# ayotoasset/AdditiveCausalExpansion

Measured on NVIDIA B200. Metric: nadam_iters_per_sec, higher is better.
Workload: dtype f64

## Files before the change

additivecausalexpansion_b200/csrc/uut_i8.cuh:

```cuda
#pragma once
#include "common.cuh"

namespace ace {

namespace oz {
constexpr int NMOD = 16;
constexpr int MOD[NMOD] = {256, 255, 253, 251, 247, 241, 239, 233, 229, 227, 223, 217, 211, 199, 197, 193};
constexpr int BM = 128, BN = 256, BK = 32;
constexpr int CPB = TB / BK;
constexpr int STAGES = 8;
constexpr int A_BYTES = BM * BK, B_BYTES = BN * BK;
constexpr int STAGE_BYTES = A_BYTES + B_BYTES;
constexpr size_t SMEM_BYTES = 1024 + (size_t)STAGES * STAGE_BYTES + 128;
static_assert(2 * SMEM_BYTES <= 227 * 1024 && 3 * SMEM_BYTES > 228 * 1024, "exactly two CTAs per SM");
constexpr int TMEM_COLS = BN;
constexpr int THREADS = 192;
constexpr int MAX_N = 65408;
static_assert((long)128 * 128 * MAX_N <= 2147483647L, "INT32 accumulators may overflow");
constexpr uint32_t IDESC = (2u << 4) | (1u << 7) | (1u << 10) | ((uint32_t)(BN >> 3) << 17) | ((uint32_t)(BM >> 4) << 24);

constexpr int crt_bits(int n_pad) { return n_pad <= 16384 ? 55 : 54; }
constexpr unsigned __int128 crt_half_range() {
  unsigned __int128 p = 1;
  for (int t = 0; t < NMOD; ++t) p *= (unsigned)MOD[t];
  return p / 2;
}
static_assert(((unsigned __int128)16384 << (2 * 55)) < crt_half_range(), "CRT range at b = 55");
static_assert(((unsigned __int128)MAX_N << (2 * 54)) < crt_half_range(), "CRT range at b = 54");

__host__ __device__ inline size_t block_off(int nb, int t, int rb, int c) {
  const long nc = (long)nb * CPB;
  const long per_plane = (long)nb * nc - (long)CPB * nb * (nb - 1) / 2;
  const long off = (long)rb * nc - (long)CPB * rb * (rb - 1) / 2 + (c - (long)CPB * rb);
  return ((size_t)t * per_plane + off) * (size_t)(BM * BK);
}
__host__ __device__ inline size_t slot_bytes(int nb) { return block_off(nb, 1, 0, 0); }
inline size_t plane_bytes(int nb) { return block_off(nb, NMOD + 1, 0, 0); }
__host__ __device__ inline size_t res_off(int ti, int tj) { return ((size_t)ti * (ti + 1) / 2 + tj) * (size_t)(TB * TB); }
inline long product_tiles(int nb) { return (long)(nb / 2) * (nb / 2 + 1) + (nb & 1) * (nb / 2 + 1); }

struct Tables {
  int m[NMOD];
  unsigned magic[NMOD];
  int c14[NMOD], c28[NMOD], c42[NMOD];
  float mf[NMOD], rcp[NMOD];
  float inv[NMOD];
  float w[NMOD][NMOD];
  unsigned long long p8;
};

inline Tables make_tables() {
  Tables T{};
  for (int k = 0; k < NMOD; ++k) {
    const long m = MOD[k];
    T.m[k] = (int)m;
    T.magic[k] = (unsigned)(((1ull << 32) + (unsigned long long)m - 1) / (unsigned long long)m);
    T.c14[k] = (int)((1L << 14) % m);
    T.c28[k] = (int)((1L << 28) % m);
    T.c42[k] = (int)((1L << 42) % m);
    T.mf[k] = (float)m;
    T.rcp[k] = 1.0f / (float)m;
    long pk = 1;
    for (int j = 0; j < k; ++j) pk = pk * MOD[j] % m;
    long inv = 1;
    while (k > 0 && pk * inv % m != 1) ++inv;
    T.inv[k] = (float)inv;
    long pj = 1;
    for (int j = 0; j < k; ++j) {
      T.w[k][j] = (float)(pj * inv % m);
      pj = pj * MOD[j] % m;
    }
  }
  T.p8 = 1;
  for (int j = 0; j < 8; ++j) T.p8 *= (unsigned long long)MOD[j];
  return T;
}
}

__device__ __forceinline__ int oz_smod(unsigned x, const oz::Tables& T, int t) {
  const int r = (int)(x - (unsigned)T.m[t] * __umulhi(x, T.magic[t]));
  return r > (T.m[t] >> 1) ? r - T.m[t] : r;
}

__device__ __forceinline__ uint64_t oz_smem_desc(uint32_t saddr) {
  return (uint64_t)((saddr >> 4) & 0x3FFF) | ((uint64_t)(128 >> 4) << 16) | ((uint64_t)(256 >> 4) << 32) |
         (1ull << 46);
}

__device__ __forceinline__ void tc_fence_before() { asm volatile("tcgen05.fence::before_thread_sync;" ::: "memory"); }
__device__ __forceinline__ void tc_fence_after() { asm volatile("tcgen05.fence::after_thread_sync;" ::: "memory"); }

__device__ __forceinline__ void tc_mma_i8(uint32_t d_tmem, uint64_t adesc, uint64_t bdesc, uint32_t accumulate) {
  asm volatile(
      "{\n.reg .pred p;\nsetp.ne.b32 p, %4, 0;\n"
      "tcgen05.mma.cta_group::1.kind::i8 [%0], %1, %2, %3, p;\n}\n" ::"r"(d_tmem),
      "l"(adesc), "l"(bdesc), "r"(oz::IDESC), "r"(accumulate)
      : "memory");
}

__device__ __forceinline__ void tc_commit(uint64_t* bar) {
  asm volatile("tcgen05.commit.cta_group::1.mbarrier::arrive::one.shared::cluster.b64 [%0];" ::"r"(smem_u32(bar))
               : "memory");
}

__device__ __forceinline__ void tc_ld16(uint32_t taddr, uint32_t (&v)[16]) {
  asm volatile(
      "tcgen05.ld.sync.aligned.32x32b.x16.b32 {%0,%1,%2,%3,%4,%5,%6,%7,%8,%9,%10,%11,%12,%13,%14,%15}, [%16];"
      : "=r"(v[0]), "=r"(v[1]), "=r"(v[2]), "=r"(v[3]), "=r"(v[4]), "=r"(v[5]), "=r"(v[6]), "=r"(v[7]), "=r"(v[8]),
        "=r"(v[9]), "=r"(v[10]), "=r"(v[11]), "=r"(v[12]), "=r"(v[13]), "=r"(v[14]), "=r"(v[15])
      : "r"(taddr)
      : "memory");
}

__device__ __forceinline__ double oz_u(const double* A, long ld, const double* DU, int rb, int cb, int r, int kk) {
  return (cb == rb) ? DU[(size_t)rb * TB * TB + r + (size_t)kk * TB] : A[(size_t)rb * TB + r + (size_t)(cb * TB + kk) * ld];
}

__global__ void __launch_bounds__(128) oz_rowmax_kernel(const double* __restrict__ A, long ld,
                                                        const double* __restrict__ DU,
                                                        unsigned long long* __restrict__ rowmax) {
  const int cb = blockIdx.x, rb = blockIdx.y, r = threadIdx.x;
  if (cb < rb) return;
  double m = 0.0;
#pragma unroll 8
  for (int kk = 0; kk < TB; ++kk) m = fmax(m, fabs(oz_u(A, ld, DU, rb, cb, r, kk)));
  atomicMax(rowmax + rb * TB + r, (unsigned long long)__double_as_longlong(m));
}

__global__ void __launch_bounds__(128) oz_split_kernel(const double* __restrict__ A, long ld,
                                                       const double* __restrict__ DU,
                                                       const unsigned long long* __restrict__ rowmax, int nb, int b,
                                                       const __grid_constant__ oz::Tables T,
                                                       int8_t* __restrict__ planes, int* __restrict__ ex) {
  using namespace oz;
  const int cb = blockIdx.x, rb = blockIdx.y, r = threadIdx.x;
  if (cb < rb) return;
  const double m = __longlong_as_double((long long)rowmax[rb * TB + r]);
  int e = 0;
  if (m > 0.0) frexp(m, &e);
  if (cb == rb) ex[rb * TB + r] = e;
  const double scale = ldexp(1.0, b - e);
#pragma unroll 1
  for (int q = 0; q < TB / 16; ++q) {
    uint32_t w[NMOD][4];
#pragma unroll
    for (int t = 0; t < NMOD; ++t) w[t][0] = w[t][1] = w[t][2] = w[t][3] = 0u;
#pragma unroll
    for (int x16 = 0; x16 < 16; ++x16) {
      const long long a = __double2ll_rn(rint(oz_u(A, ld, DU, rb, cb, r, q * 16 + x16) * scale));
      const unsigned long long ua = (unsigned long long)(a < 0 ? -a : a);
      const unsigned q0 = (unsigned)ua & 0x3FFFu, q1 = (unsigned)(ua >> 14) & 0x3FFFu,
                     q2 = (unsigned)(ua >> 28) & 0x3FFFu, q3 = (unsigned)(ua >> 42);
      const int sh = 8 * (x16 & 3);
      w[0][x16 >> 2] |= ((uint32_t)a & 0xffu) << sh;
#pragma unroll
      for (int t = 1; t < NMOD; ++t) {
        const int s = oz_smod(q0 + q1 * (unsigned)T.c14[t] + q2 * (unsigned)T.c28[t] + q3 * (unsigned)T.c42[t], T, t);
        w[t][x16 >> 2] |= ((uint32_t)(a < 0 ? -s : s) & 0xffu) << sh;
      }
    }
    const int c = cb * CPB + q / 2;
    const size_t in_blk = (size_t)(r >> 3) * 256 + (q & 1) * 128 + (r & 7) * 16;
#pragma unroll
    for (int t = 0; t < NMOD; ++t)
      *reinterpret_cast<uint4*>(planes + block_off(nb, t + 1, rb, c) + in_blk) =
          make_uint4(w[t][0], w[t][1], w[t][2], w[t][3]);
  }
}

__global__ void __launch_bounds__(oz::THREADS, 2) uut_i8_mod_kernel(int8_t* __restrict__ planes, int nb, int slot,
                                                                    int m, double inv_m) {
  using namespace oz;
  extern __shared__ unsigned char smem_raw[];
  unsigned char* sm = reinterpret_cast<unsigned char*>((reinterpret_cast<uintptr_t>(smem_raw) + 1023) & ~uintptr_t(1023));
  uint64_t* full = reinterpret_cast<uint64_t*>(sm + (size_t)STAGES * STAGE_BYTES);
  uint64_t* empty = full + STAGES;
  uint64_t* done = empty + STAGES;
  uint32_t* tmem_slot = reinterpret_cast<uint32_t*>(done + 1);
  const int warp = threadIdx.x >> 5, lane = threadIdx.x & 31;

  int ti, tj2;
  {
    const long L = blockIdx.x;
    long q = (long)((sqrt(4.0 * (double)L + 1.0) - 1.0) * 0.5);
    while (q * (q + 1) > L) --q;
    while ((q + 1) * (q + 2) <= L) ++q;
    const long rem = L - q * (q + 1);
    ti = (int)(2 * q + rem / (q + 1));
    tj2 = (int)(rem % (q + 1));
  }
  const int jb0 = 2 * tj2;
  const bool has1 = jb0 + 1 <= ti;
  const int jb1 = has1 ? jb0 + 1 : jb0;
  const int c_begin = ti * CPB, nchunks = nb * CPB - c_begin;
  const int8_t* src = planes;

  if (threadIdx.x == 0) {
    for (int s = 0; s < STAGES; ++s) {
      mbar_init(&full[s], 1);
      mbar_init(&empty[s], 1);
    }
    mbar_init(done, 1);
    fence_mbar_init();
  }
  if (warp == 1) {
    asm volatile("tcgen05.alloc.cta_group::1.sync.aligned.shared::cta.b32 [%0], %1;" ::"r"(smem_u32(tmem_slot)),
                 "r"(TMEM_COLS)
                 : "memory");
    asm volatile("tcgen05.relinquish_alloc_permit.cta_group::1.sync.aligned;" ::: "memory");
  }
  tc_fence_before();
  __syncthreads();
  tc_fence_after();
  const uint32_t tmem = *tmem_slot;

  if (warp == 0) {
    if (lane == 0) {
      for (int it = 0; it < nchunks; ++it) {
        const int s = it % STAGES;
        mbar_wait(&empty[s], ((it / STAGES) & 1) ^ 1);
        mbar_arrive_expect_tx(&full[s], STAGE_BYTES);
        unsigned char* st = sm + (size_t)s * STAGE_BYTES;
        const int c = c_begin + it;
        tma_bulk_g2s(st, src + block_off(nb, slot + 1, ti, c), A_BYTES, &full[s]);
        tma_bulk_g2s(st + A_BYTES, src + block_off(nb, slot + 1, jb0, c), A_BYTES, &full[s]);
        tma_bulk_g2s(st + 2 * A_BYTES, src + block_off(nb, slot + 1, jb1, c), A_BYTES, &full[s]);
      }
    }
    __syncwarp();
  } else if (warp == 1) {
    if (lane == 0) {
      for (int it = 0; it < nchunks; ++it) {
        const int s = it % STAGES;
        mbar_wait(&full[s], (it / STAGES) & 1);
        tc_fence_after();
        const uint32_t a0 = smem_u32(sm + (size_t)s * STAGE_BYTES);
        tc_mma_i8(tmem, oz_smem_desc(a0), oz_smem_desc(a0 + A_BYTES), it > 0 ? 1u : 0u);
        tc_commit(&empty[s]);
      }
      tc_commit(done);
    }
    __syncwarp();
  } else {
    mbar_wait(done, 0);
    tc_fence_after();
    const int q = warp & 3;
    const int r = q * 32 + lane;
    const uint32_t trow = tmem + ((uint32_t)(q * 32) << 16);
    int8_t* dst = planes + block_off(nb, slot, 0, 0) + (size_t)r * TB;
#pragma unroll 1
    for (int jc = 0; jc < (has1 ? BN : TB) / 32; ++jc) {
      uint32_t v[2][16];
      tc_ld16(trow + (uint32_t)(jc * 32), v[0]);
      tc_ld16(trow + (uint32_t)(jc * 32 + 16), v[1]);
      asm volatile("tcgen05.wait::ld.sync.aligned;" ::: "memory");
      uint32_t pk[8];
#pragma unroll
      for (int j = 0; j < 32; ++j) {
        const int x = (int)v[j >> 4][j & 15];
        int res;
        if (m == 256) {
          res = x;
        } else {
          res = x - m * (int)rint((double)x * inv_m);
        }
        if ((j & 3) == 0) pk[j >> 2] = 0u;
        pk[j >> 2] |= ((uint32_t)res & 0xffu) << (8 * (j & 3));
      }
      uint4* o = reinterpret_cast<uint4*>(dst + res_off(ti, jb0 + (jc >> 2)) + (jc & 3) * 32);
      o[0] = make_uint4(pk[0], pk[1], pk[2], pk[3]);
      o[1] = make_uint4(pk[4], pk[5], pk[6], pk[7]);
    }
  }
  tc_fence_before();
  __syncthreads();
  if (warp == 1) {
    tc_fence_after();
    asm volatile("tcgen05.dealloc.cta_group::1.sync.aligned.b32 %0, %1;" ::"r"(tmem), "r"(TMEM_COLS) : "memory");
  }
}

__device__ __forceinline__ float oz_i2f(int x) { return __int_as_float(0x4B400000 + x) - 0x1.8p23f; }
__device__ __forceinline__ int oz_f2i(float x) { return __float_as_int(x + 0x1.8p23f) - 0x4B400000; }

__device__ __forceinline__ double oz_crt(const int (&res)[oz::NMOD], const oz::Tables& T, int scale_exp) {
  using namespace oz;
  float v[NMOD];
  v[0] = oz_i2f(res[0]);
#pragma unroll
  for (int k = 1; k < NMOD; ++k) {
    float s = oz_i2f(res[k]) * T.inv[k];
#pragma unroll
    for (int j = 0; j < k; ++j) s = fmaf(-v[j], T.w[k][j], s);
    float r = fmaf(-T.mf[k], rintf(s * T.rcp[k]), s);
    const float h = 0.5f * T.mf[k];
    r = r > h ? r - T.mf[k] : r;
    r = r < -h ? r + T.mf[k] : r;
    v[k] = r;
  }
  unsigned long long ulo = (unsigned long long)(long long)oz_f2i(v[7]);
  unsigned long long uhi = (unsigned long long)(long long)oz_f2i(v[NMOD - 1]);
#pragma unroll
  for (int k = 6; k >= 0; --k) ulo = ulo * (unsigned)T.m[k] + (unsigned long long)(long long)oz_f2i(v[k]);
#pragma unroll
  for (int k = NMOD - 2; k >= 8; --k) uhi = uhi * (unsigned)T.m[k] + (unsigned long long)(long long)oz_f2i(v[k]);
  const __int128 x = (__int128)(long long)uhi * (__int128)T.p8 + (__int128)(long long)ulo;
  const bool neg = x < 0;
  const unsigned __int128 u = neg ? (unsigned __int128)(-x) : (unsigned __int128)x;
  const unsigned long long hi = (unsigned long long)(u >> 64), lo = (unsigned long long)u;
  double d;
  if (hi == 0) {
    d = ldexp(__ull2double_rn(lo), scale_exp);
  } else {
    const int z = __clzll((long long)hi);
    const unsigned long long top = z ? (hi << z) | (lo >> (64 - z)) : hi;
    const unsigned long long rest = lo << z;
    d = ldexp(__ull2double_rn(top | (rest != 0 ? 1ull : 0ull)), scale_exp + 64 - z);
  }
  return neg ? -d : d;
}

__global__ void __launch_bounds__(256) oz_crt_kernel(const int8_t* __restrict__ planes, const int* __restrict__ ex,
                                                     int nb, int b, const __grid_constant__ oz::Tables T,
                                                     double* __restrict__ C, long ldc) {
  using namespace oz;
  __shared__ double tile[32][TB + 1];
  int ti, tj;
  {
    const long L = blockIdx.x;
    long t = (long)((sqrt(8.0 * (double)L + 1.0) - 1.0) * 0.5);
    while (t * (t + 1) / 2 > L) --t;
    while ((t + 1) * (t + 2) / 2 <= L) ++t;
    ti = (int)t;
    tj = (int)(L - t * (t + 1) / 2);
  }
  const size_t sb = slot_bytes(nb);
  const int8_t* blk = planes + res_off(ti, tj);
  const int tid = threadIdx.x, rr = tid >> 3, c0 = (tid & 7) * 16;
  const int i0 = ti * TB, j0 = tj * TB;
#pragma unroll 1
  for (int r0 = 0; r0 < TB; r0 += 32) {
    const int r = r0 + rr;
    uint4 rv[NMOD];
#pragma unroll
    for (int t = 0; t < NMOD; ++t) rv[t] = *reinterpret_cast<const uint4*>(blk + t * sb + (size_t)r * TB + c0);
    const int ei = ex[i0 + r];
#pragma unroll 1
    for (int j = 0; j < 16; ++j) {
      int res[NMOD];
#pragma unroll
      for (int t = 0; t < NMOD; ++t) {
        const uint32_t wv = j < 4 ? rv[t].x : j < 8 ? rv[t].y : j < 12 ? rv[t].z : rv[t].w;
        res[t] = (int)(int8_t)(wv >> (8 * (j & 3)));
      }
      tile[rr][c0 + j] = oz_crt(res, T, ei + ex[j0 + c0 + j] - 2 * b);
    }
    __syncthreads();
#pragma unroll 4
    for (int k = tid; k < 32 * TB; k += 256) {
      const int a = k >> 7, c = k & (TB - 1);
      C[(size_t)(i0 + r0 + a) * ldc + j0 + c] = tile[a][c];
    }
    if (ti != tj) {
#pragma unroll 4
      for (int k = tid; k < 32 * TB; k += 256) {
        const int c = k >> 5, a = k & 31;
        C[(size_t)(j0 + c) * ldc + i0 + r0 + a] = tile[a][c];
      }
    }
    __syncthreads();
  }
}

struct OzWork {
  int8_t* planes = nullptr;
  unsigned long long* rowmax = nullptr;
  int* ex = nullptr;
};

inline int configure_uut_i8_kernel() {
  ACE_CUDA(cudaFuncSetAttribute(uut_i8_mod_kernel, cudaFuncAttributeMaxDynamicSharedMemorySize, (int)oz::SMEM_BYTES));
  return 0;
}

inline int launch_uut_i8(const OzWork& o, const double* A, const double* DU, int nb, double* C, cudaStream_t st) {
  using namespace oz;
  if ((long)nb * TB > MAX_N) {
    set_error("uut_i8: n_pad beyond the CRT range bound");
    return -2;
  }
  if (!o.planes || !o.rowmax || !o.ex) {
    set_error("uut_i8: residue-plane workspace not allocated");
    return -2;
  }
  static const Tables T = make_tables();
  const long ld = (long)nb * TB;
  const int b = crt_bits((int)ld);
  ACE_CUDA(cudaMemsetAsync(o.rowmax, 0, sizeof(unsigned long long) * (size_t)ld, st));
  const dim3 g2(nb, nb);
  oz_rowmax_kernel<<<g2, TB, 0, st>>>(A, ld, DU, o.rowmax);
  ACE_CUDA(cudaGetLastError());
  oz_split_kernel<<<g2, TB, 0, st>>>(A, ld, DU, o.rowmax, nb, b, T, o.planes, o.ex);
  ACE_CUDA(cudaGetLastError());
  const long tiles = product_tiles(nb);
  for (int t = 0; t < NMOD; ++t) {
    uut_i8_mod_kernel<<<(unsigned)tiles, THREADS, SMEM_BYTES, st>>>(o.planes, nb, t, MOD[t], 1.0 / MOD[t]);
    ACE_CUDA(cudaGetLastError());
  }
  oz_crt_kernel<<<(unsigned)((long)nb * (nb + 1) / 2), 256, 0, st>>>(o.planes, o.ex, nb, b, T, C, ld);
  ACE_CUDA(cudaGetLastError());
  return 0;
}

}
```

Baseline: 8.075.

## Compute residues with paired fp32 FMA magic-number rounding in split and mod kernels

Replaces the integer magic-division modular reductions in the residue split kernel and the fp64 rint-based reduction in the TMEM epilogue with packed float2 FMA arithmetic. Values are decomposed into 14-bit pieces via fp64 magic-constant tricks, combined with signed residue constants and reduced using a biased round-to-nearest, so the low byte of the float bits is the residue. Bytes are packed with byte_perm instead of shift/or loops. This is meant to cut integer-multiply and fp64 cost in these phases, at the risk of subtle exactness errors if fp32 intermediate ranges are exceeded.

```diff
diff --git a/additivecausalexpansion_b200/csrc/uut_i8.cuh b/additivecausalexpansion_b200/csrc/uut_i8.cuh
--- a/additivecausalexpansion_b200/csrc/uut_i8.cuh
+++ b/additivecausalexpansion_b200/csrc/uut_i8.cuh
@@ -41,8 +41,8 @@
 
 struct Tables {
   int m[NMOD];
-  unsigned magic[NMOD];
-  int c14[NMOD], c28[NMOD], c42[NMOD];
+  float2 s_c14[NMOD], s_c28[NMOD], s_c42[NMOD];
+  float2 s_rcp[NMOD], s_nm[NMOD];
   float mf[NMOD], rcp[NMOD];
   float inv[NMOD];
   float w[NMOD][NMOD];
@@ -54,10 +54,12 @@
   for (int k = 0; k < NMOD; ++k) {
     const long m = MOD[k];
     T.m[k] = (int)m;
-    T.magic[k] = (unsigned)(((1ull << 32) + (unsigned long long)m - 1) / (unsigned long long)m);
-    T.c14[k] = (int)((1L << 14) % m);
-    T.c28[k] = (int)((1L << 28) % m);
-    T.c42[k] = (int)((1L << 42) % m);
+    auto smod = [m](long x) { x %= m; return (float)(x > m / 2 ? x - m : x); };
+    T.s_c14[k] = make_float2(smod(1L << 14), smod(1L << 14));
+    T.s_c28[k] = make_float2(smod(1L << 28), smod(1L << 28));
+    T.s_c42[k] = make_float2(smod(1L << 42), smod(1L << 42));
+    T.s_rcp[k] = make_float2(1.0f / (float)m, 1.0f / (float)m);
+    T.s_nm[k] = make_float2(-(float)m, -(float)m);
     T.mf[k] = (float)m;
     T.rcp[k] = 1.0f / (float)m;
     long pk = 1;
@@ -77,9 +79,14 @@
 }
 }
 
-__device__ __forceinline__ int oz_smod(unsigned x, const oz::Tables& T, int t) {
-  const int r = (int)(x - (unsigned)T.m[t] * __umulhi(x, T.magic[t]));
-  return r > (T.m[t] >> 1) ? r - T.m[t] : r;
+constexpr float OZ_MAGIC = 0x1.8p23f;
+__device__ __forceinline__ float oz_i2f(int x) { return __int_as_float(0x4B400000 + x) - OZ_MAGIC; }
+__device__ __forceinline__ int oz_f2i(float x) { return __float_as_int(x + OZ_MAGIC) - 0x4B400000; }
+__device__ __forceinline__ float2 oz_f2(float x) { return make_float2(x, x); }
+
+__device__ __forceinline__ float2 oz_smod2_biased(float2 s, float2 rcp, float2 nm) {
+  const float2 q = __fadd2_rn(__ffma2_rn(s, rcp, oz_f2(OZ_MAGIC)), oz_f2(-OZ_MAGIC));
+  return __fadd2_rn(__ffma2_rn(q, nm, s), oz_f2(OZ_MAGIC));
 }
 
 __device__ __forceinline__ uint64_t oz_smem_desc(uint32_t saddr) {
@@ -127,6 +134,17 @@
   atomicMax(rowmax + rb * TB + r, (unsigned long long)__double_as_longlong(m));
 }
 
+__device__ __forceinline__ void oz_pieces(double v, float (&p)[4], uint32_t& low) {
+  const double th = fma(v, 0x1p-28, 0x1.8p52);
+  const int hi = __double2loint(th);
+  const int lo = __double2loint(fma(-(th - 0x1.8p52), 0x1p28, v) + 0x1.8p52);
+  low = (uint32_t)lo;
+  p[0] = __int_as_float(0x4B400000 | (lo & 0x3FFF)) - OZ_MAGIC;
+  p[1] = oz_i2f(lo >> 14);
+  p[2] = __int_as_float(0x4B400000 | (hi & 0x3FFF)) - OZ_MAGIC;
+  p[3] = oz_i2f(hi >> 14);
+}
+
 __global__ void __launch_bounds__(128) oz_split_kernel(const double* __restrict__ A, long ld,
                                                        const double* __restrict__ DU,
                                                        const unsigned long long* __restrict__ rowmax, int nb, int b,
@@ -135,6 +153,7 @@
   using namespace oz;
   const int cb = blockIdx.x, rb = blockIdx.y, r = threadIdx.x;
   if (cb < rb) return;
+  const size_t in_row = (size_t)(r >> 3) * 256 + (r & 7) * 16;
   const double m = __longlong_as_double((long long)rowmax[rb * TB + r]);
   int e = 0;
   if (m > 0.0) frexp(m, &e);
@@ -144,32 +163,38 @@
   for (int q = 0; q < TB / 16; ++q) {
     uint32_t w[NMOD][4];
 #pragma unroll
-    for (int t = 0; t < NMOD; ++t) w[t][0] = w[t][1] = w[t][2] = w[t][3] = 0u;
-#pragma unroll
-    for (int x16 = 0; x16 < 16; ++x16) {
-      const long long a = __double2ll_rn(rint(oz_u(A, ld, DU, rb, cb, r, q * 16 + x16) * scale));
-      const unsigned long long ua = (unsigned long long)(a < 0 ? -a : a);
-      const unsigned q0 = (unsigned)ua & 0x3FFFu, q1 = (unsigned)(ua >> 14) & 0x3FFFu,
-                     q2 = (unsigned)(ua >> 28) & 0x3FFFu, q3 = (unsigned)(ua >> 42);
-      const int sh = 8 * (x16 & 3);
-      w[0][x16 >> 2] |= ((uint32_t)a & 0xffu) << sh;
+    for (int x4 = 0; x4 < 4; ++x4) {
+      float p[4][4];
+      uint32_t low[4];
+#pragma unroll
+      for (int x = 0; x < 4; ++x) oz_pieces(oz_u(A, ld, DU, rb, cb, r, q * 16 + x4 * 4 + x) * scale, p[x], low[x]);
+      w[0][x4] = __byte_perm(__byte_perm(low[0], low[1], 0x0040), __byte_perm(low[2], low[3], 0x0040), 0x5410);
 #pragma unroll
       for (int t = 1; t < NMOD; ++t) {
-        const int s = oz_smod(q0 + q1 * (unsigned)T.c14[t] + q2 * (unsigned)T.c28[t] + q3 * (unsigned)T.c42[t], T, t);
-        w[t][x16 >> 2] |= ((uint32_t)(a < 0 ? -s : s) & 0xffu) << sh;
+        uint32_t bits[4];
+#pragma unroll
+        for (int h = 0; h < 2; ++h) {
+          float2 s = make_float2(p[2 * h][0], p[2 * h + 1][0]);
+          s = __ffma2_rn(make_float2(p[2 * h][1], p[2 * h + 1][1]), T.s_c14[t], s);
+          s = __ffma2_rn(make_float2(p[2 * h][2], p[2 * h + 1][2]), T.s_c28[t], s);
+          s = __ffma2_rn(make_float2(p[2 * h][3], p[2 * h + 1][3]), T.s_c42[t], s);
+          const float2 rb2 = oz_smod2_biased(s, T.s_rcp[t], T.s_nm[t]);
+          bits[2 * h] = __float_as_uint(rb2.x);
+          bits[2 * h + 1] = __float_as_uint(rb2.y);
+        }
+        w[t][x4] = __byte_perm(__byte_perm(bits[0], bits[1], 0x0040), __byte_perm(bits[2], bits[3], 0x0040), 0x5410);
       }
     }
     const int c = cb * CPB + q / 2;
-    const size_t in_blk = (size_t)(r >> 3) * 256 + (q & 1) * 128 + (r & 7) * 16;
 #pragma unroll
     for (int t = 0; t < NMOD; ++t)
-      *reinterpret_cast<uint4*>(planes + block_off(nb, t + 1, rb, c) + in_blk) =
+      *reinterpret_cast<uint4*>(planes + block_off(nb, t + 1, rb, c) + (q & 1) * 128 + in_row) =
           make_uint4(w[t][0], w[t][1], w[t][2], w[t][3]);
   }
 }
 
 __global__ void __launch_bounds__(oz::THREADS, 2) uut_i8_mod_kernel(int8_t* __restrict__ planes, int nb, int slot,
-                                                                    int m, double inv_m) {
+                                                                    int m, float rcp_m, float c16) {
   using namespace oz;
   extern __shared__ unsigned char smem_raw[];
   unsigned char* sm = reinterpret_cast<unsigned char*>((reinterpret_cast<uintptr_t>(smem_raw) + 1023) & ~uintptr_t(1023));
@@ -256,16 +281,25 @@
       asm volatile("tcgen05.wait::ld.sync.aligned;" ::: "memory");
       uint32_t pk[8];
 #pragma unroll
-      for (int j = 0; j < 32; ++j) {
-        const int x = (int)v[j >> 4][j & 15];
-        int res;
-        if (m == 256) {
-          res = x;
-        } else {
-          res = x - m * (int)rint((double)x * inv_m);
+      for (int j4 = 0; j4 < 8; ++j4) {
+        uint32_t bits[4];
+#pragma unroll
+        for (int h = 0; h < 4; h += 2) {
+          const int x0 = (int)v[j4 >> 2][(j4 & 3) * 4 + h], x1 = (int)v[j4 >> 2][(j4 & 3) * 4 + h + 1];
+          if (m == 256) {
+            bits[h] = (uint32_t)x0;
+            bits[h + 1] = (uint32_t)x1;
+          } else {
+            float2 s = __fadd2_rn(make_float2(__int_as_float(0x4B400000 | (x0 & 0xFFFF)),
+                                              __int_as_float(0x4B400000 | (x1 & 0xFFFF))),
+                                  oz_f2(-OZ_MAGIC));
+            s = __ffma2_rn(make_float2(oz_i2f(x0 >> 16), oz_i2f(x1 >> 16)), oz_f2(c16), s);
+            const float2 rb2 = oz_smod2_biased(s, oz_f2(rcp_m), oz_f2(-(float)m));
+            bits[h] = __float_as_uint(rb2.x);
+            bits[h + 1] = __float_as_uint(rb2.y);
+          }
         }
-        if ((j & 3) == 0) pk[j >> 2] = 0u;
-        pk[j >> 2] |= ((uint32_t)res & 0xffu) << (8 * (j & 3));
+        pk[j4] = __byte_perm(__byte_perm(bits[0], bits[1], 0x0040), __byte_perm(bits[2], bits[3], 0x0040), 0x5410);
       }
       uint4* o = reinterpret_cast<uint4*>(dst + res_off(ti, jb0 + (jc >> 2)) + (jc & 3) * 32);
       o[0] = make_uint4(pk[0], pk[1], pk[2], pk[3]);
@@ -279,9 +313,6 @@
     asm volatile("tcgen05.dealloc.cta_group::1.sync.aligned.b32 %0, %1;" ::"r"(tmem), "r"(TMEM_COLS) : "memory");
   }
 }
-
-__device__ __forceinline__ float oz_i2f(int x) { return __int_as_float(0x4B400000 + x) - 0x1.8p23f; }
-__device__ __forceinline__ int oz_f2i(float x) { return __float_as_int(x + 0x1.8p23f) - 0x4B400000; }
 
 __device__ __forceinline__ double oz_crt(const int (&res)[oz::NMOD], const oz::Tables& T, int scale_exp) {
   using namespace oz;
@@ -404,7 +435,9 @@
   ACE_CUDA(cudaGetLastError());
   const long tiles = product_tiles(nb);
   for (int t = 0; t < NMOD; ++t) {
-    uut_i8_mod_kernel<<<(unsigned)tiles, THREADS, SMEM_BYTES, st>>>(o.planes, nb, t, MOD[t], 1.0 / MOD[t]);
+    const int c16 = (1 << 16) % MOD[t];
+    uut_i8_mod_kernel<<<(unsigned)tiles, THREADS, SMEM_BYTES, st>>>(o.planes, nb, t, MOD[t], 1.0f / (float)MOD[t],
+                                                                    (float)(c16 > MOD[t] / 2 ? c16 - MOD[t] : c16));
     ACE_CUDA(cudaGetLastError());
   }
   oz_crt_kernel<<<(unsigned)((long)nb * (nb + 1) / 2), 256, 0, st>>>(o.planes, o.ex, nb, b, T, C, ld);
```

Measured after the change: 8.125, median of 6. About the same (+0.6%).
